# medical-genomics-group/hydra

Hardware: AMD Instinct MI355X
Metric: Gibbs markers/sec/iter (higher is better)
Workload: dtype f64

## Files before the change

### hydra_amd/capi.py

```python
import ctypes as C
import os
import numpy as np

_HERE = os.path.dirname(os.path.abspath(__file__))
LIB_PATH = os.path.join(_HERE, "libhgibbs.so")

ABI_SYMBOLS = [
    "hgibbs_last_error", "hgibbs_version", "hgibbs_create", "hgibbs_destroy", "hgibbs_comm_unique_id",
    "hgibbs_comm_init", "hgibbs_comm_init_external", "hgibbs_p2p_export", "hgibbs_p2p_import", "hgibbs_load_bed", "hgibbs_synth_bed", "hgibbs_dims", "hgibbs_get_bed",
    "hgibbs_marker_stats", "hgibbs_set_residual", "hgibbs_get_residual", "hgibbs_reduce_eps", "hgibbs_add_scalar",
    "hgibbs_update_marker", "hgibbs_dot_marker", "hgibbs_set_covariates", "hgibbs_cov_dot", "hgibbs_cov_update",
    "hydra_chain_set_covariates", "hydra_chain_gamma", "hgibbs_set_components", "hydra_chain_restore",
    "hydra_rng_to_boost_words", "hydra_rng_from_boost_words", "hydra_rng_shuffle", "hgibbs_set_model", "hgibbs_set_beta", "hgibbs_get_beta",
    "hgibbs_beta_sqnorm", "hgibbs_sweep", "hgibbs_set_option", "hgibbs_last_sweep_stats", "hgibbs_stream_ceiling", "hgibbs_debug_times", "hgibbs_resident_trace", "hydra_chain_create",
    "hydra_chain_destroy", "hydra_chain_iterate", "hydra_chain_state", "hydra_chain_csv_line", "hydra_chain_order",
    "hydra_chain_last_nnz", "hgibbs_score", "hgibbs_last_score_ms", "hgibbs_ld", "hgibbs_last_ld_ms",
    "hgibbs_ld_scores", "hgibbs_last_ld_scores_ms",
    "hgibbs_marker_dots", "hgibbs_last_marker_dots_ms", "hgibbs_king", "hgibbs_king_pairs", "hgibbs_king_pairs_get", "hgibbs_last_king_ms",
    "hgibbs_pca", "hgibbs_last_pca_ms", "hgibbs_region_var", "hgibbs_last_region_var_ms",
    "hgibbs_grm", "hgibbs_grm_info", "hgibbs_last_grm_ms",
    "hgibbs_grand_seed", "hgibbs_grand_next", "hgibbs_ars_sample", "hgibbs_w_init", "hgibbs_w_marker_stats", "hgibbs_w_set_model",
    "hgibbs_w_reduce", "hgibbs_w_refresh_vi", "hgibbs_w_get_vi", "hgibbs_w_marker_sums", "hgibbs_w_sweep", "hgibbs_w_last_sweep_stats", "hgibbs_w_ars_device_probe",
    "hgibbs_w_get_beta", "hgibbs_w_set_beta", "hydraw_chain_create", "hydraw_chain_destroy", "hydraw_chain_set_covariates",
    "hydraw_chain_reseed_ars", "hydraw_chain_iterate", "hydraw_chain_state", "hydraw_chain_gamma", "hydraw_chain_order",
    "hydraw_chain_last_nnz", "hydraw_chain_csv_line", "hydraw_chain_restore",
]


class RngState(C.Structure):
    _fields_ = [("x", C.c_uint32 * 624), ("idx", C.c_uint32)]


class SweepStats(C.Structure):
    _fields_ = [("launches", C.c_uint64), ("nnz_updates", C.c_uint64), ("device_ms", C.c_double),
                ("kernel_ms_avg", C.c_double), ("carried_columns", C.c_uint64), ("working_launches", C.c_uint64),
                ("accepted_markers", C.c_uint64), ("streamed_columns", C.c_uint64), ("tiles_per_workgroup_min", C.c_uint32),
                ("tiles_per_workgroup_max", C.c_uint32), ("engine", C.c_uint32), ("walker", C.c_uint32), ("eps_sum_drift", C.c_double),
                ("rounds", C.c_uint64), ("events", C.c_uint64), ("advances", C.c_uint64), ("chunks", C.c_uint64), ("refolds", C.c_uint64), ("pivots", C.c_uint64), ("predicted", C.c_uint64), ("shader_mhz", C.c_double),
                ("ticks", C.c_uint64 * 16), ("refill", C.c_uint32), ("reserved_", C.c_uint32)]


class PcaReport(C.Structure):
    _fields_ = [("iters_run", C.c_int32), ("m_used", C.c_uint32), ("ritz_change", C.c_double), ("resid", C.c_double * 32)]


class RestartState(C.Structure):
    _fields_ = [("iteration", C.c_uint32), ("sigmaE", C.c_double), ("mu", C.c_double),
                ("sigmaG", C.POINTER(C.c_double)), ("estPi", C.POINTER(C.c_double)), ("beta", C.POINTER(C.c_double)),
                ("components", C.POINTER(C.c_int32)), ("eps", C.POINTER(C.c_double)), ("order", C.POINTER(C.c_int32)),
                ("gamma", C.POINTER(C.c_double)), ("xI", C.POINTER(C.c_int32)), ("rng", RngState)]


class GrandState(C.Structure):
    _fields_ = [("r", C.c_int32 * 31), ("f", C.c_int32), ("b", C.c_int32)]


class WSweepStats(C.Structure):
    _fields_ = [("launches", C.c_uint64), ("nnz_updates", C.c_uint64), ("ars_draws", C.c_uint64), ("ars_evals", C.c_uint64),
                ("device_ms", C.c_double), ("sums_kernel_ms", C.c_double)]


class WModelDesc(C.Structure):
# ... 489 lines not shown
        order = np.ascontiguousarray(order, dtype=np.int32)
        sigmaG = np.ascontiguousarray(sigmaG, dtype=np.float64)
        estPi = np.ascontiguousarray(estPi, dtype=np.float64)
        adaV = np.ascontiguousarray(adaV, dtype=np.uint8)
        cass = np.zeros((self.G, self.K), dtype=np.int32)
        nnz = C.c_uint64()
        check(self.L.hgibbs_sweep(self.h, _ip(order), float(sigmaE), _dp(sigmaG), _dp(estPi), _u8(adaV), C.byref(rng),
                                  _ip(cass), C.byref(nnz)))
        return cass, nnz.value

    def resident_trace(self):
        out = np.zeros((10, 4096), dtype=np.uint64)
        check(self.L.hgibbs_resident_trace(self.h, out.ctypes.data_as(C.POINTER(C.c_uint64)), out.size))
        return out

    def sweep_stats(self):
        s = SweepStats()
        check(self.L.hgibbs_last_sweep_stats(self.h, C.byref(s)))
        return {"launches": s.launches, "nnz_updates": s.nnz_updates, "device_ms": s.device_ms,
                "kernel_ms_avg": s.kernel_ms_avg, "carried_columns": s.carried_columns, "working_launches": s.working_launches,
                "accepted_markers": s.accepted_markers, "streamed_columns": s.streamed_columns,
                "tiles_per_workgroup_min": s.tiles_per_workgroup_min, "tiles_per_workgroup_max": s.tiles_per_workgroup_max,
                "engine": s.engine, "walker": s.walker, "refill": s.refill, "eps_sum_drift": s.eps_sum_drift, "rounds": s.rounds, "events": s.events,
                "advances": s.advances, "chunks": s.chunks, "refolds": s.refolds, "pivots": s.pivots, "predicted": s.predicted, "shader_mhz": s.shader_mhz, "ticks": list(s.ticks)}


class Chain:

    def __init__(self, dev, y, mS=None, groups=None, seed=1222, shuffle=1):
        self.dev = dev
        self.L = dev.L
        if mS is None:
            mS = np.array([[0.0, 0.0001, 0.001, 0.01]])
        self.mS = np.ascontiguousarray(mS, dtype=np.float64)
        self.G, self.K = self.mS.shape
        self.groups = None if groups is None else np.ascontiguousarray(groups, dtype=np.int32)
        y = np.ascontiguousarray(y, dtype=np.float64)
        assert y.shape[0] == dev.n_global
        d = ModelDesc(seed, shuffle, self.G, self.K, _ip(self.groups) if self.groups is not None else None, _dp(self.mS))
        self.h = C.c_void_p()
        check(self.L.hydra_chain_create(dev.h, C.byref(d), _dp(y), C.byref(self.h)))
        dev.G, dev.K = self.G, self.K

    def __del__(self):
        try:
            if self.h:
                self.L.hydra_chain_destroy(self.h)
# ... 214 lines not shown
```

### hydra_amd/csrc/hg_resident.hip.h

```cpp
#pragma once

#include "hg_sweep.hip.h"

namespace hg {

constexpr int RS_WAVES = 8;
constexpr int RS_BLOCK = RS_WAVES * WAVE;
constexpr int RS_BMAX = 256;
constexpr int RS_NSH = 8;
constexpr int RS_RSH = 8;
constexpr int RS_GROW = 1024;
constexpr int RS_CROW = 1024;
constexpr int RS_RB = 2 * RS_BMAX;
constexpr int RS_MSG = 16;
constexpr int RS_PMAX = 4;
constexpr int RS_PFIRE = 16;
constexpr int RS_NB = 256;
constexpr int RS_TRACE = 4096;
constexpr int RS_TMAX = 2;
constexpr uint32_t RS_ONE = 1u << 24;
constexpr uint32_t RS_LOW = RS_ONE - 1u;
constexpr unsigned long long RS_ONE64 = 1ull << 56;
constexpr int RS_GFX = 32;
constexpr int RS_FG = 4, RS_FN = 256;
// ... 7 lines not shown
    double dbeta;
};
__host__ __device__ inline uint32_t rs_msg_check(uint32_t seq, uint32_t lo, uint32_t hi)
{
    uint32_t x = seq * 0x9E3779B1u ^ lo ^ (hi * 0x85EBCA77u);
    x ^= x >> 16;
    return x & 0xffffu;
}
constexpr unsigned long long RS_RONE = 1ull << 56;
__host__ __device__ inline unsigned long long rs_raw_value(unsigned long long d) { return (unsigned long long)((long long)(d << 8) >> 8); }
__host__ __device__ inline uint32_t rs_raw_count(unsigned long long d) { return (uint32_t)((d - rs_raw_value(d)) >> 56) & 0xffu; }
__host__ __device__ inline uint32_t rs_window_end(uint32_t C, uint32_t B, uint32_t M, uint32_t mask)
{
    const uint32_t e = (C + B) & ~mask;
    return e < M ? e : M;
}
__host__ __device__ inline uint32_t rs_msg_word0(uint32_t kf, uint32_t ncons, uint32_t seq, uint32_t lo, uint32_t hi) { return (kf << 28) | (rs_msg_check(seq, lo, hi) << 12) | ncons; }

struct ResState {
    uint32_t cursor, rng_idx, error, pad;
    unsigned long long rounds, events, advances, nnz, chunks, refolds, pivots, predicted;
    unsigned long long shader_ticks, wall_ticks;
    unsigned long long t[16];
};

struct ResParams {
    const uint8_t* bed;
    uint64_t stride;
    double* eps;
    uint32_t n_pad, n_local, M;
    double n_minus_1, n_total, eps_sum;
    const int32_t* order;
    const double* s_mave;
    const double* s_mstd;
    const double* s_bold;
    const int32_t* s_ga;
    double* beta;
    int32_t* comp;
    double* acum;
    int32_t* cass;
    int K, GK;
    const double* denom;
    const double* logpi;
    const double* hlog;
    const double* sdk;
    double i_2sigE;
// ... 9 lines not shown
    unsigned long long* racc2;
    unsigned long long* gacc64;
    const unsigned long long* counts;
    unsigned long long* pacc;
    ResMsg* msg;
    ResState* state;
    double fx_scale, fx_unscale;
    unsigned long long timeout;
    unsigned long long* progress;
    unsigned long long rdv_timeout;
    unsigned long long* trace;
    int dbg;
    int pivots;
    int unused_;
    int early_advance;
    uint32_t wend_mask;
    int announce;
    int walker;
    const uint32_t* pred;
    int all_ada;
    int nranks, rank;
    unsigned char* mbox[RX_MAXR];
    unsigned long long sweep_id;
};

constexpr uint32_t RX_RING = 1024;
constexpr size_t RX_GBOX = 0;
constexpr size_t RX_RBOX = RX_GBOX + (size_t)RX_MAXR * 2 * RS_BMAX * 16;
constexpr size_t RX_HBOX = RX_RBOX + (size_t)RX_MAXR * RX_RING * 32;
constexpr size_t RX_BYTES = RX_HBOX + (size_t)RX_MAXR * 2 * 8;
__device__ __forceinline__ unsigned long long* rx_gbox(unsigned char* mb, int src, uint32_t par) { return reinterpret_cast<unsigned long long*>(mb + RX_GBOX) + ((size_t)src * 2 + par) * RS_BMAX * 2; }
__device__ __forceinline__ unsigned long long* rx_rbox(unsigned char* mb, int src) { return reinterpret_cast<unsigned long long*>(mb + RX_RBOX) + (size_t)src * RX_RING * 4; }
__device__ __forceinline__ unsigned long long* rx_hbox(unsigned char* mb, int src) { return reinterpret_cast<unsigned long long*>(mb + RX_HBOX) + (size_t)src * 2; }
__device__ __forceinline__ unsigned long long rx_rtag(unsigned long long sweep, uint32_t batch) { return (0x80000000ull | ((sweep & 0x7ffull) << 20) | (unsigned long long)(batch & 0xfffffu)) << 32; }

typedef uint32_t u4_t __attribute__((ext_vector_type(4)));
typedef __attribute__((address_space(4))) uint32_t rs_cu32;
__device__ __forceinline__ u4_t rs_load16(const void* p)
{
    u4_t v;
    asm volatile("global_load_dwordx4 %0, %1, off sc1\n\ts_waitcnt vmcnt(0)" : "=v"(v) : "v"(p) : "memory");
    return v;
}
__device__ __forceinline__ void rs_lds_barrier() { asm volatile("s_waitcnt lgkmcnt(0)\n\ts_barrier" ::: "memory"); }
__device__ __forceinline__ void rs_store16(void* p, u4_t v) { asm volatile("global_store_dwordx4 %0, %1, off sc1" ::"v"(p), "v"(v) : "memory"); }
__device__ __forceinline__ double rs_readlane(double v, int l)
// ... 403 lines not shown
        last = (kf & RS_LAST) != 0u;
        ncons = (uint32_t)tag & 0xfffu;
        lap(0);
        if (timing) p.trace[4 * RS_TRACE + seq % RS_TRACE] = wall_clock64();
    };
    for (;;) {
        const bool ann = kind == RS_ANNOUNCE;
        const bool upd = kind == RS_EVENT || kind == RS_PIVOT || kind == RS_ANNOUNCED;
        const bool with_gram = kind == RS_EVENT || ann || (kind == RS_ANNOUNCED && !gram_sent);
        if (DBG && wg == 0 && tid == 0) p.progress[1] = ((unsigned long long)seq << 8) | 1u;
        const uint32_t q = C + ncons - 1u;
        const uint32_t Cn = ann ? C : C + ncons;
        const uint32_t Sn = rs_window_end(Cn, B, M, p.wend_mask);
        const uint32_t nnew = Sn - Sx;
        uint32_t count_w = (Sn > (uint32_t)wave ? (Sn - (uint32_t)wave + 7u) / 8u : 0u) - nk;
        cols_landed();

        if (upd || ann) {
            const uint32_t slotq = q & bmask;
            uint32_t xq[T];
#pragma unroll
            for (int t = 0; t < T; ++t) xq[t] = ring[slotq * 64u * T + (uint32_t)lane * T + t];
            const double2 mq = meta[slotq];
            if (upd && tid < 16) {
                const double av = mq.x, sd = mq.y, db = dbeta;
                const double v0 = -(av * sd * db), v1 = db * (1.0 - av) * sd, v2 = db * (2.0 - av) * sd;
                auto addend = [&](uint32_t c) { return 0.0 + ((c == 0u) ? v0 : ((c == 1u) ? v1 : ((c == 3u) ? v2 : 0.0))); };
                tab[tid] = make_double2(addend((uint32_t)tid & 3u), addend(((uint32_t)tid >> 2) & 3u));
            }

            if (with_gram) rs_gram_terms<T, MISS>(p, ring, meta, wg, wave, lane, q, Sx, bmask, nev, xq, mq);
            if (with_gram) ++nev;
            lap(2);
            if (timing) p.trace[6 * RS_TRACE + seq % RS_TRACE] = wall_clock64();
            rs_lds_barrier();
            if (upd) {
#pragma unroll
                for (int t = 0; t < T; ++t) apply_update16_lds(xq[t], tab, e[t]);
                eps_to_lds();
            }
            lap(1);
            if (timing) p.trace[5 * RS_TRACE + seq % RS_TRACE] = wall_clock64();
        }
        gram_sent = ann;
        if (ann) {
            take_message(true);
            if (kind == RS_ABORT) break;
            continue;
        }

        if constexpr (MISS) {
            if (upd) asm volatile("s_waitcnt lgkmcnt(0)\n\ts_barrier" ::: "memory");
        }
        const uint32_t round_k0 = nk;
        uint32_t done_k0 = nk, done_m = 0;
        while (count_w) {
            if (done_m) cols_landed();
            const uint32_t m = count_w < (uint32_t)RS_PF ? count_w : (uint32_t)RS_PF;
            const int32_t ids = rs_lane_ids();
// ... 1315 lines not shown
```

### hydra_amd/csrc/hg_streamer2.hip.h

```cpp
#pragma once

namespace hg {

constexpr int RL_NG = 8;
constexpr int RL_VGPR_LIMIT = 200;
constexpr int RL_VGPR_LIMIT4 = 208;
constexpr int RL_TMAX = 4;
constexpr int RL_EX = 44;
constexpr uint32_t RL_BLK = 144;
typedef int rl_v4i __attribute__((ext_vector_type(4)));

__host__ __device__ constexpr size_t rl_meta_off() { return 512; }
__host__ __device__ constexpr size_t rl_acc_off(uint32_t B) { return 512 + (size_t)B * 16; }
__host__ __device__ constexpr size_t rl_acc2_off(uint32_t B) { return 512 + (size_t)B * 24; }
__host__ __device__ constexpr size_t rl_zero_off(uint32_t B) { return 512 + (size_t)B * 32; }
__host__ __device__ constexpr size_t rl_digit_off(uint32_t B) { return rl_zero_off(B) + 64; }
__host__ __device__ constexpr int rl_image_blocks(int T) { return 8 * T < 16 ? 8 * T : 16; }
__host__ __device__ constexpr size_t rl_ring_off(uint32_t B, int T) { return rl_digit_off(B) + (size_t)RS_WAVES * rl_image_blocks(T) * RL_BLK; }
__host__ __device__ constexpr size_t rl_streamer_lds(uint32_t B, int T) { return rl_ring_off(B, T) + (size_t)B * 256 * T; }
static_assert(rl_streamer_lds(RS_BMAX, RS_TMAX) <= 160 * 1024 && rl_streamer_lds(RS_BMAX / 2, RL_TMAX) <= 160 * 1024,
              "the largest window at the most tiles per workgroup fits the 160 KB of LDS of a compute unit");

#define RL_SET_LIST(X) X(0, 224, 225, 226, 227, 200, 201, 216) X(1, 228, 229, 230, 231, 202, 203, 217) X(2, 232, 233, 234, 235, 204, 205, 218) X(3, 236, 237, 238, 239, 206, 207, 219) \
    X(4, 240, 241, 242, 243, 208, 209, 220) X(5, 244, 245, 246, 247, 210, 211, 221) X(6, 248, 249, 250, 251, 212, 213, 222) X(7, 252, 253, 254, 255, 214, 215, 223)
// ... 312 lines not shown
        ncons = (uint32_t)tag & 0xfffu;
        lap(0);
        if (timing) p.trace[4 * RS_TRACE + seq % RS_TRACE] = wall_clock64();
    };

    for (;;) {
        const bool ann = kind == RS_ANNOUNCE;
        const bool upd = kind == RS_EVENT || kind == RS_PIVOT || kind == RS_ANNOUNCED;
        const bool with_gram = kind == RS_EVENT || ann || (kind == RS_ANNOUNCED && !gram_sent);
        if (DBG && wg == 0 && tid == 0) p.progress[1] = ((unsigned long long)seq << 8) | 1u;
        const uint32_t q = C + ncons - 1u;
        const uint32_t Cn = ann ? C : C + ncons;
        const uint32_t Sn = rs_window_end(Cn, B, M, p.wend_mask);
        const uint32_t nnew = Sn - Sx;
        cols_landed();

        if (upd || ann) {
            const uint32_t slotq = q & bmask;
            uint32_t xq[T];
#pragma unroll
            for (int t = 0; t < T; ++t) xq[t] = ring[slotq * 64u * T + (uint32_t)lane * T + t];
            const uint32_t xqe = ring[slotq * 64u * T + (uint32_t)wave * 8u * T + bw];
            const double2 mq = meta[slotq];
            if (upd && tid < 4) {
                const double av = mq.x, sd = mq.y, db = dbeta;
                const double v0 = -(av * sd * db), v1 = db * (1.0 - av) * sd, v2 = db * (2.0 - av) * sd;
                tab1[tid] = 0.0 + (tid == 0 ? v0 : (tid == 1 ? v1 : (tid == 3 ? v2 : 0.0)));
            }
            if (with_gram) rs_gram_terms<T, MISS>(p, ring, meta, wg, wave, lane, q, Sx, bmask, nev, xq, mq);

            if (with_gram) ++nev;
            lap(2);
            if (timing) p.trace[6 * RS_TRACE + seq % RS_TRACE] = wall_clock64();
            rs_lds_barrier();
            if (upd) {
#pragma unroll
                for (int s = 0; s < ND; ++s) {
                    const double add = tab1[(xqe >> (2u * eb[s])) & 3u];
                    e[s] += ev[s] ? add : 0.0;
                }
                digits_to_operands();
            }
            lap(1);
            if (timing) p.trace[5 * RS_TRACE + seq % RS_TRACE] = wall_clock64();
        }
        gram_sent = ann;
        if (ann) {
            take_message(true);
            if (kind == RS_ABORT) break;
            continue;
        }

        if (nnew) {
            const uint32_t G0 = Sx >> 4, G1 = (Sn - 1u) >> 4;
            for (uint32_t gb = G0; gb <= G1; gb += (uint32_t)NG) {
                if (gb != G0) cols_landed();
                auto one = [&](auto rtag) __attribute__((always_inline)) {
                    constexpr int r = decltype(rtag)::value;
// ... 117 lines not shown
```

### hydra_amd/csrc/hg_walker2.hip.h

```cpp
#pragma once

namespace hg {

constexpr int W2_NBLK = 4;
constexpr uint32_t W2_RING = W2_NBLK * MT_N;
constexpr uint32_t W2_RR = 1024;
constexpr uint32_t W2_EV = 64;
constexpr uint32_t W2_PRED = 1024;
constexpr uint32_t W2_NB = 256;
constexpr int W2_NCH = 4;
constexpr uint32_t W2_NREC = 8;

enum {
    S_FPUB = 0,
    S_MPUB,
    S_CPUB,
    S_SEQPUB,
    S_RECSEQ,
    S_BLK,
    S_GPOS,
    S_PLD,
    S_PCUR,
    S_RDONE,
    S_EVN,
// ... 5 lines not shown
    S_NWORDS = 32
};
enum {
    R_TYPE = 0,
    R_Q,
    R_CN,
    R_SXO,
    R_SXN,
    R_FD,
    R_SEQ,
    R_PIN,
    R_PIQ,
    R_NEV,
    R_GPOSR,
    R_PFN,
    R_DB = 12,
    R_MQ = 14,
    R_SQ = 16,
    R_GSQ = 18,
    R_NMQ = 20,
    R_WORDS = 32
};
enum { RT_EXTEND = 0, RT_ADVANCE = 1, RT_PIVOT = 2, RT_EVENT = 3, RT_END = 4 };
enum { W2_ST_ROUNDS = 0, W2_ST_EVENTS, W2_ST_ADV, W2_ST_NNZ, W2_ST_CHUNKS, W2_ST_REFOLD, W2_ST_PIVOTS, W2_ST_PRED, W2_ST_ANN };

#define W2_ARRAYS(X)                                                                                                                          \
    X(double, tq, (size_t)W2_RING)         \
    X(double, zig_nx, 130)                                                                                                                    \
    X(double, zig_ny, 130)                                                                                                                    \
    X(double, htab, (size_t)4 * HT_LDS)                                                                                                       \
    X(double, qtab, (size_t)2 * HT_LDS)                                                                                                       \
    X(double, ftab, (size_t)RS_FG * (RS_FN + 1))                                                                                              \
    X(double, fscale, RS_FG)                                                                                                                  \
    X(double, mave, MR)                                                                               \
    X(double, mstd, MR)                                                                                                                       \
    X(double, bold, MR)                                                                                                                       \
    X(double, gsum, MR)                                                                                                     \
    X(double, nmis, MR)                                                                                                                       \
    X(double, dpr, Bz)                                                                               \
    X(double, rnum, (size_t)W2_RR)                                                                      \
    X(double, ev_bnew, (size_t)W2_EV)                                                                                                         \
    X(unsigned long long, rprev, (size_t)RS_RB)                                \
    X(unsigned long long, rprev2, (size_t)RS_RB)                                                                                              \
    X(unsigned long long, pprev, (size_t)2 * RS_RB)                                                                                           \
    X(unsigned long long, rloc, Bz)        \
    X(unsigned long long, rloc2, Bz)                                                                       \
    X(uint32_t, rpushed, Bz)                                                                             \
// ... 84 lines not shown
    const Walk2Off off = walk2_offsets(B);
    uint32_t lb = (uint32_t)__builtin_amdgcn_readfirstlane((int)(uint32_t)(uintptr_t)(W2_LDS unsigned char*)hg_smem);
    asm volatile("" : "+s"(lb));
    W2_LDS unsigned char* const lbase = (W2_LDS unsigned char*)(uintptr_t)lb;
#define W2_X(type, name, count) sh.name = (W2_LDS type*)(lbase + off.name);
    W2_ARRAYS(W2_X)
#undef W2_X
    return sh;
}

#define W2_BEXPR pr.B
#define W2_PIVEXPR (pr.pivots != 0)
#define W2_PROLOGUE \
    const int tid = threadIdx.x, lane = tid & 63; \
    const int wave = __builtin_amdgcn_readfirstlane(tid >> 6); \
    const uint32_t B = W2_BEXPR, bmask = B - 1u, M = pr.M; \
    const uint32_t MR = 2u * B, mrmask = MR - 1u; \
    const int K = pr.K, GK = pr.GK; \
    const uint32_t W = pr.W, nsh = pr.nsh, rsh = pr.rsh; \
    const double n_total = pr.n_total, n_minus_1 = pr.n_minus_1, i_2sigE = pr.i_2sigE, eps_sum = pr.eps_sum, fx_unscale = pr.fx_unscale; \
    const unsigned long long timeout = pr.timeout; \
    const bool pivots = W2_PIVEXPR; \
    const uint32_t early_advance = (uint32_t)pr.early_advance; \
    const bool announce = pr.announce != 0 && !pivots; \
    const uint32_t rng_idx0 = pr.rng_idx; \
    ResMsg* const msg = pr.msg; \
    ResState* const state = pr.state; \
    unsigned long long* const trace = pr.trace; \
    unsigned long long* const progress = pr.progress; \
    const uint32_t* const gpred = pr.pred; \
    const double* const zig_ex = pr.zig.ex; \
    const double* const zig_ey = pr.zig.ey; \
    const Walk2Lds sh = walk2_lds(B); \
    const uint32_t cntG[2] = {W / nsh + (W % nsh ? 1u : 0u), W / nsh}; \
    const uint32_t cntR[2] = {W / rsh + (W % rsh ? 1u : 0u), W / rsh}; \
    const uint32_t wend_mask = pr.wend_mask; \
    const int nranks = pr.nranks, rank = pr.rank; \
    const unsigned long long sweep_id = pr.sweep_id; \
    const uint32_t Sx0 = rs_window_end(0u, B, M, wend_mask); \
    const uint32_t m0 = MR < M ? MR : M; \
    auto stage_meta = [&](uint32_t j) { \
        const uint32_t ms = j & mrmask; \
        const int ga = pr.s_ga[j]; \
        const int mk = pr.order[j]; \
        sh.marker[ms] = mk; \
        sh.ga[ms] = ga; \
        sh.bold[ms] = pr.s_bold[j]; \
        sh.mave[ms] = pr.s_mave[j]; \
        sh.mstd[ms] = pr.s_mstd[j]; \
        if constexpr (MISS) { \
            const unsigned long long* cn = pr.counts + 3ull * (unsigned long long)mk; \
            sh.gsum[ms] = (double)(cn[0] + 2ull * cn[1]); \
            sh.nmis[ms] = (double)cn[2]; \
        } \
    }; \
    auto tq_of = [&](uint32_t word) { \
        const double prob = (double)mt_temper(word) * (1.0 / 4294967296.0); \
        return log(1.0 / prob - 1.0) - 1e-9; \
    }; \
    auto aborted = [&]() { return w2_ld(sh.sw + S_ABORT) != 0u; }; \
    auto ended = [&]() { return w2_ld(sh.sw + S_END) != 0u; };

template <int DBG, int MISS, int BC, int RANKS, int DECIDE, int PIV>
__device__ __attribute__((noinline)) void w2_chain(const ResParams& prg)
{
    typedef const __attribute__((address_space(4))) ResParams w2_cparams;
    const unsigned long long pga = (unsigned long long)(uintptr_t)&prg;
    const unsigned long long pgu = ((unsigned long long)(uint32_t)__builtin_amdgcn_readfirstlane((int)(uint32_t)(pga >> 32)) << 32) |
                                   (uint32_t)__builtin_amdgcn_readfirstlane((int)(uint32_t)pga);
    w2_cparams& pr = *(w2_cparams*)(uintptr_t)pgu;
#undef W2_BEXPR
#define W2_BEXPR (BC ? (uint32_t)BC : pr.B)
#undef W2_PIVEXPR
#define W2_PIVEXPR (PIV != 0)
    W2_PROLOGUE
#undef W2_BEXPR
#define W2_BEXPR pr.B
#undef W2_PIVEXPR
#define W2_PIVEXPR (pr.pivots != 0)
    __builtin_amdgcn_s_setprio(3);
    constexpr bool decider = DECIDE != 0;
    const uint32_t nch = B >= 64u ? B / 64u : 1u;
    const uint32_t slot = (uint32_t)wave * 64u + (uint32_t)lane;
    const bool son = slot < B;
    const uint32_t sl = son ? slot : 0u;
    double dpr = 0.0, dp = 0.0, mave = 0.0, mstd = 0.0, boldn = 0.0, fsc = 0.0, gsm = 0.0, nms = 0.0;
    uint32_t fof = 0, sbt = 0, spi = 0;
    bool prd = false;
    uint32_t C = 0, Sx = 0, Fs = 0, base = 0, gposr = rng_idx0 % W2_RING;
    uint32_t gpa32[RS_NSH], gpb32[RS_NSH];
    unsigned long long gpa64[RS_NSH], gpb64[RS_NSH];
#pragma unroll
    for (int r = 0; r < RS_NSH; ++r) {
        gpa32[r] = gpb32[r] = 0u;
        gpa64[r] = gpb64[r] = 0ull;
    }
    typedef const __attribute__((address_space(1))) uint32_t* w2_g32;
    typedef const __attribute__((address_space(1))) unsigned long long* w2_g64;
    const w2_g32 gacc = (w2_g32)pr.gacc;
    const w2_g64 gacc64 = (w2_g64)pr.gacc64;
    uint32_t rno = 0;

    uint32_t seq = 0, nev = 0, pi = 0, evn = 0, pf_n = 0, gpos = rng_idx0, blk = 1u;
    uint32_t rdone_seen = 0, wpub_seen = 0, evw_seen = 0, pld_seen = W2_PRED, fpub_seen = 0, mpub_seen = m0;
    unsigned long long cm[W2_NCH] = {0ull, 0ull, 0ull, 0ull};
    uint32_t stat = 0;
    auto count = [&](uint32_t bits) { stat += (bits >> (uint32_t)lane) & 1u; };
    uint32_t err = 0;
    bool failed = false;
    unsigned long long tacc[8] = {0ull, 0ull, 0ull, 0ull, 0ull, 0ull, 0ull, 0ull};
    unsigned long long tmark = DBG ? wall_clock64() : 0ull;
    auto lap = [&](int i) {
        if (DBG && decider) {
            const unsigned long long now = wall_clock64();
            tacc[i] += now - tmark;
            tmark = now;
        }
    };
    auto pos_of_slot = [&](uint32_t s, uint32_t c) { return c + ((s - c) & bmask); };
    uint32_t nspin = 0;
    auto spin_fail = [&](unsigned long long t0) {
        if (aborted()) return true;
        if (wall_clock64() - t0 > timeout || ((++nspin & 1023u) == 0u && w2_uni((uint32_t)(__hip_atomic_load(progress + 2, HG_RLX_AGENT) != 0ull)) != 0u)) {
            if (lane == 0) w2_st(sh.sw + S_ABORT, 1u);
            return true;
        }
        return false;
// ... 332 lines not shown
                    if ((uint32_t)t <= nch && qs == 0xffffffffu) {
                        uint32_t i = i0 + (uint32_t)t;
                        i = i >= nch ? i - nch : i;
                        unsigned long long mm = i == 0u ? cm[0] : (i == 1u ? cm[1] : (i == 2u ? cm[2] : cm[3]));
                        if (t == 0) mm &= ~lowm;
                        if ((uint32_t)t == nch) mm &= lowm;
                        if (mm) qs = i * 64u + (uint32_t)(__ffsll((long long)mm) - 1);
                    }
                }
                qs = w2_uni(qs);
                if (qs == 0xffffffffu) break;
                const uint32_t qc = pos_of_slot(qs, C);
                const uint32_t qi = qs >> 6, ql = qs & 63u;
                const uint32_t ms = qc & mrmask;
                uint32_t upos = gposr + (qc - C);
                upos = upos >= W2_RING ? upos - W2_RING : upos;
                const double bold_v = sh.bold[ms], num = sh.rnum[qc & (W2_RR - 1u)];
                const double cmq_v = sh.mave[ms], csq_v = sh.mstd[ms], cgsq_v = MISS ? sh.gsum[ms] : 0.0, cnmq_v = MISS ? sh.nmis[ms] : 0.0;
                const int ga_v = sh.ga[ms];
                const uint32_t word_v = sh.mt[upos];
                const uint32_t zp1 = upos + 1u == W2_RING ? 0u : upos + 1u, zp2 = zp1 + 1u == W2_RING ? 0u : zp1 + 1u;
                const uint32_t zw1 = sh.mt[zp1], zw2 = sh.mt[zp2];
                const double bold = w2_uni(bold_v);
                if (announce && !announced && bold != 0.0 && qc + 1u < Sx && (seq + 6u <= (uint32_t)RS_MSG || rdone_seen >= seq + 6u - (uint32_t)RS_MSG)) {
                    if (lane == 0) rs_store16(msg + ((seq + 1u) % RS_MSG), rs_u4(rs_msg_word0((uint32_t)RS_ANNOUNCE, qc - C + 1u, seq + 1u, 0u, 0u), seq + 1u, 0u, 0u));
                    announced = true;
                }
                const uint32_t zleft = blk * (uint32_t)MT_N - (gpos + (qc - C) + 1u);
                double z;
                bool zfast;
                {
                    const uint32_t u1 = mt_temper(w2_uni(zw1)), u2 = mt_temper(w2_uni(zw2));
                    int zi = (int)(u1 & 0xffu);
                    double r = (double)(u1 >> 8) * (1.0 / 16777216.0);
                    r += (double)(u2 & 0x1fffffffu);
                    r *= (1.0 / 536870912.0);
                    const int sign = (zi & 1) * 2 - 1;
                    zi >>= 1;
                    const double x = r * sh.zig_nx[zi];
                    zfast = zleft >= 2u && x < sh.zig_nx[zi + 1];
                    z = x * sign;
                }
                const int g0 = w2_uni(ga_v & 0x0fffffff) * K;
                const double prob = (double)mt_temper(word_v) * (1.0 / 4294967296.0);
                double Lm = 0.0, mk = 0.0, sdl = 0.0;
                {
                    const int lk = lane < K ? lane : 0;
// ... 37 lines not shown
                if (k > 0) {
                    const double mean_k = rs_readlane(mk, k), sd_k = rs_readlane(sdl, k);
                    if (zfast) {
                        bnew = z * sd_k + mean_k;
                        consumed = 2u;
                    } else {
                        if (lane == 0) {
                            RingGen g{sh.mt, zp1, zleft, 0u, 0u};
                            const ZigLds zt{sh.zig_nx, sh.zig_ny, zig_ex, zig_ey};
                            bnew = norm_rng_sd(g, zt, mean_k, sd_k);
                            consumed = g.n;
                            gerr = g.err;
                        }
                        bnew = w2_uni(bnew);
                        consumed = (uint32_t)__builtin_amdgcn_readlane((int)consumed, 0);
                        gerr = (uint32_t)__builtin_amdgcn_readlane((int)gerr, 0);
                    }
                }
                if (gerr) {
                    err = gerr;
                    failed = true;
                    break;
                }
                if (k != 0 || bold != 0.0) {
                    found = true;
                    q_mq = w2_uni(cmq_v);
                    q_sq = w2_uni(csq_v);
                    q_gsq = w2_uni(cgsq_v);
                    q_nmq = w2_uni(cnmq_v);
                    qpos = qc;
                    q_k = k;
                    q_bnew = bnew;
                    q_bold = bold;
                    q_consumed = consumed;
                    break;
                }
                const unsigned long long bit = 1ull << ql;
                if (qi == 0u) cm[0] &= ~bit;
                else if (qi == 1u) cm[1] &= ~bit;
                else if (qi == 2u) cm[2] &= ~bit;
                else cm[3] &= ~bit;
            }
        }
        lap(3);
        if (failed) break;
        const uint32_t early_thr = early_advance;
        const bool early = !found && Fs < Sx && early_thr != 0u && Fs - C >= early_thr;
        if (!found && Fs < Sx && !early) {
            count(1u << W2_ST_REFOLD);
            if (!wait_seen(fpub_seen, S_FPUB, Fs + 1u)) break;
            lap(0);
            publish(RT_EXTEND, 0u, C, Sx, Sx, fpub_seen < Sx ? fpub_seen : Sx, 0u, 0.0, 0.0, 0.0, 0.0, 0.0);
            continue;
        }
        const uint32_t ncons = found ? qpos - C + 1u : (early ? Fs - C : Sx - C);
        const uint32_t Cn = C + ncons;
        const uint32_t Sn = rs_window_end(Cn, B, M, wend_mask);
        const double dbeta = found ? q_bold - q_bnew : 0.0;
        const bool changed = found && dbeta != 0.0;
        const bool is_event = changed || announced;
        const bool predicted = found && q_bold != 0.0;
        bool pivot = false;
        if (PIV && is_event && predicted && pf_n < (uint32_t)RS_PFIRE)
            pivot = qpos + 1u >= Sx || pi - w2_uni(sh.bl_pi[w2_uni(sh.batch[(qpos + 1u) & bmask]) % W2_NB]) < (uint32_t)RS_PMAX;
        lap(6);
        {
            const uint32_t a = w2_uni(fc_rdone), b = w2_uni(fc_wpub), c = w2_uni(fc_evw);
            rdone_seen = a > rdone_seen ? a : rdone_seen;
            wpub_seen = b > wpub_seen ? b : wpub_seen;
            evw_seen = c > evw_seen ? c : evw_seen;
        }
        if (seq + 6u > (uint32_t)RS_MSG && !wait_seen(rdone_seen, S_RDONE, seq + 6u - (uint32_t)RS_MSG)) break;
        if (Cn + B > W2_RR && !wait_seen(wpub_seen, S_WPUB, Cn + B - W2_RR)) break;
        if (evn + 2u > W2_EV && !wait_seen(evw_seen, S_EVW, evn + 2u - W2_EV)) break;
        lap(2);
        ++seq;
        if (lane == 0) {
            const uint32_t kf = (pivot ? (uint32_t)RS_PIVOT : (announced ? (uint32_t)RS_ANNOUNCED : (is_event ? (uint32_t)RS_EVENT : (uint32_t)RS_ADVANCE))) | (Cn >= M ? (uint32_t)RS_LAST : 0u);
            const unsigned long long db = (unsigned long long)__double_as_longlong(dbeta);
            if (DBG) {
                w2_gst(trace + (2 * RS_TRACE + (seq - 1u) % RS_TRACE), wall_clock64());
                w2_gst(trace + (3 * RS_TRACE + (seq - 1u) % RS_TRACE), ncons);
                w2_gst(trace + (0 * RS_TRACE + seq % RS_TRACE), wall_clock64());
                if (!(is_event && !pivot)) w2_gst(trace + (1 * RS_TRACE + seq % RS_TRACE), wall_clock64());
            }
            rs_store16(msg + (seq % RS_MSG), rs_u4(rs_msg_word0(kf, ncons, seq, (uint32_t)db, (uint32_t)(db >> 32)), seq, (uint32_t)db, (uint32_t)(db >> 32)));
        }
        count((1u << W2_ST_ROUNDS) | (is_event ? (1u << W2_ST_EVENTS) | (changed ? 1u << W2_ST_NNZ : 0u) | (predicted ? 1u << W2_ST_PRED : 0u) |
                                                      (announced ? 1u << W2_ST_ANN : 0u)
                                                : 1u << W2_ST_ADV) |
              (pivot ? 1u << W2_ST_PIVOTS : 0u));
        const bool round_trip = is_event && !pivot;
        if (round_trip) ++nev;
        const double mq = q_mq, sq = q_sq, gsq = q_gsq, nmq = q_nmq;
        const uint32_t evr = evn;
        if (found) ++evn;
        const uint32_t piq = pi;
        fpub_seen = w2_ld(sh.sw + S_FPUB);
        const uint32_t Fd = fpub_seen < Sx ? fpub_seen : Sx;
        if (PIV && pivot && Fs < Sx) {
            if (lane == 0) {
                sh.pf_pos[pf_n] = qpos;
                sh.pf_msg[pf_n] = seq;
                sh.pf_pi[pf_n] = pi;
                sh.pf_val[3 * pf_n] = dbeta;
                sh.pf_val[3 * pf_n + 1] = mq;
                sh.pf_val[3 * pf_n + 2] = sq;
            }
            ++pf_n;
        }
        if (PIV && predicted) ++pi;
        gpos += ncons + q_consumed;
        const uint32_t rtype = found ? (pivot ? (uint32_t)RT_PIVOT : (is_event ? (uint32_t)RT_EVENT : (uint32_t)RT_ADVANCE)) : (uint32_t)RT_ADVANCE;
        if (lane == 0) {
// ... 29 lines not shown
        if (C < M) {
            ++seq;
            if (lane == 0) {
                w2_st(sh.sw + S_ABORT, 1u);
                rs_store16(msg + (seq % RS_MSG), rs_u4(rs_msg_word0((uint32_t)RS_ABORT, 0u, seq, 0u, 0u), seq, 0u, 0u));
                atomicMax(&state->error, err ? err : 3u);
            }
        }
        publish(RT_END, 0u, C, Sx, Sx, 0u, 0u, 0.0, 0.0, 0.0, 0.0, 0.0);
        if (lane == 0) {
            w2_st(sh.sw + S_GPOS, gpos);
            w2_lds_done();
            w2_st(sh.sw + S_END, 1u);
            state->cursor = C;
            auto st = [&](int i) { return (uint32_t)__builtin_amdgcn_readlane((int)stat, i); };
            state->rounds = st(W2_ST_ROUNDS);
            state->events = st(W2_ST_EVENTS);
            state->advances = st(W2_ST_ADV);
            state->nnz = st(W2_ST_NNZ);
            state->chunks = st(W2_ST_CHUNKS);
            state->refolds = st(W2_ST_REFOLD);
            state->pivots = st(W2_ST_PIVOTS) + st(W2_ST_ANN);
            state->predicted = st(W2_ST_PRED);
            if (DBG)
                for (int i = 0; i < 8; ++i) state->t[i] = tacc[i];
        }
    }
}

template <int MISS, int RANKS>
__device__ __attribute__((noinline)) void w2_folder(const ResParams& pr)
{
    W2_PROLOGUE
    uint32_t Ff = 0, done = 0, fb = 0;
    unsigned long long t_idle = wall_clock64();
    auto poll_done = [&]() {
        uint32_t b = 0xffffffffu;
        if ((uint32_t)lane < rsh) b = __hip_atomic_load(pr.rcnt + (size_t)lane * RS_CROW, HG_RLX_AGENT) / cntR[(uint32_t)lane < W % rsh ? 0 : 1];
#pragma unroll
        for (int off = 32; off >= 1; off >>= 1) {
            const uint32_t o = (uint32_t)__shfl_xor((int)b, off, 64);
            b = o < b ? o : b;
        }
        done = (uint32_t)__builtin_amdgcn_readfirstlane((int)b);
        if (lane == 0) w2_st(sh.sw + S_RDONE, done);
    };
// ... 378 lines not shown
```

### hydra_amd/csrc/hgibbs.hip

```cpp
#include <hip/hip_runtime.h>
#include <rccl/rccl.h>

#include <algorithm>
#include <atomic>
#include <chrono>
#include <thread>
#include <cmath>
#include <cstdarg>
#include <cstdio>
#include <cstdlib>
#include <cstring>
#include <string>
#include <vector>

#include "../../include/hgibbs.h"
#include "hg_kernels.h"
#include "hg_sweep.hip.h"
#include "hg_resident.hip.h"

using namespace hg;

static thread_local std::string g_err;

static int fail(const char* fmt, ...)
// ... 107 lines not shown
    uint32_t cols_per_group = 4;
    int chunk = 0;
    uint32_t slices = 0;
    uint32_t ext_limit = 256;
    uint32_t max_seg = 0;
    bool gram = true;
    bool use_graph = false;
    bool force_split = false;

    int engine = 0;
    bool res_all_ada = false;
    unsigned long long res_sweep_id = 0;
    bool engine_pinned = false;
    uint32_t window = 0;
    uint32_t res_cus = 0;
    int res_walker = 0;
    bool res_attr_set[20] = {};
    bool res_dead = false;
    uint32_t res_probed_w = 0;
    unsigned long long res_probe_id = 0;
    bool res_not_resident = false;
    int res_early = 24;
    int res_announce = 1;
    int res_wend = 1;
    int res_walker2_ranks = 1;
    double eps_abs_bound = 0.0;
    int res_refill = 0;
    int res_pivots = 0;
    unsigned char* res_acc = nullptr;
    ResMsg* res_msg = nullptr;
    ResState* res_state = nullptr;
    ResState* res_state_host = nullptr;
    ResParams* res_params = nullptr;
    ResParams* res_params_host = nullptr;
    unsigned long long* res_progress = nullptr;
    unsigned long long* res_progress_host = nullptr;
    hipStream_t aux_stream = nullptr;
    unsigned long long* res_trace = nullptr;
    double res_timeout_s = 2.0;
    double res_deadline_s = 0.0;

    hgibbs_sweep_stats stats{};
    int score_sp = 0;
    int score_ranges = 0;
    double score_ms = 0.0;
    int ld_split = 0;
// ... 1082 lines not shown
    } else if (!std::strcmp(name, "ahead")) {
        if (value < -1 || value > AHEAD_MAX) return fail("ahead must be in [-1,%d] (-1 = auto)", AHEAD_MAX);
        h->ahead = (int)value;

    } else if (!std::strcmp(name, "engine")) {
        if (value < 0 || value > 2) return fail("engine must be 0 (auto), 1 (batch) or 2 (resident)");
        h->engine = (int)value;
    } else if (!std::strcmp(name, "window")) {
        if (value != 0 && (value < 8 || value > RS_BMAX || (value & (value - 1)))) return fail("window must be 0 (auto) or a power of two in [8,%d]", RS_BMAX);
        h->window = (uint32_t)value;
    } else if (!std::strcmp(name, "pivots")) {
        h->res_pivots = value != 0;
    } else if (!std::strcmp(name, "early_advance")) {
        if (value < 0 || value > 255) return fail("early_advance must be in [0,255]");
        h->res_early = (int)value;
    } else if (!std::strcmp(name, "refill")) {
        if (value < 0 || value > 2) return fail("refill must be 0 (auto), 1 (fused multiply-adds) or 2 (integer matrix products)");
        h->res_refill = (int)value;
    } else if (!std::strcmp(name, "walker2_ranks")) {
        h->res_walker2_ranks = value != 0;
    } else if (!std::strcmp(name, "window_end16")) {
        h->res_wend = value != 0;
    } else if (!std::strcmp(name, "announce")) {
        h->res_announce = value != 0;
    } else if (!std::strcmp(name, "walker")) {
        if (value < 0 || value > 2) return fail("walker must be 0 (auto), 1 (first) or 2 (second)");
        h->res_walker = (int)value;
    } else if (!std::strcmp(name, "res_cus")) {
        if (value < 0 || value > 4096) return fail("res_cus must be in [0,4096]");
        h->res_cus = (uint32_t)value;
    } else if (!std::strcmp(name, "res_deadline_ms")) {
        h->res_deadline_s = (double)value * 1e-3;
    } else if (!std::strcmp(name, "res_timeout_ms")) {
        if (value < 1) return fail("res_timeout_ms must be positive");
        h->res_timeout_s = (double)value * 1e-3;
    } else if (!std::strcmp(name, "p2p")) {
        h->p2p_enabled = value != 0;
    } else if (!std::strcmp(name, "force_split")) {
        h->force_split = value != 0;
    } else if (!std::strcmp(name, "w_kernel_timing")) {
        h->w_kernel_timing = value != 0;
    } else if (!std::strcmp(name, "debug_timing")) {
        h->debug_timing = value != 0;
    } else if (!std::strcmp(name, "chunk")) {
        h->chunk = (int)value;
    } else {
        return fail("hgibbs_set_option: unknown option '%s'", name);
// ... 208 lines not shown
    p.racc2 = reinterpret_cast<unsigned long long*>(h->res_acc + RES_RACC2_OFF);
    p.gacc64 = reinterpret_cast<unsigned long long*>(h->res_acc + RES_RACC2_OFF + RES_RACC_BYTES);
    p.counts = h->counts;
    p.msg = h->res_msg;
    p.state = h->res_state;
    {
        const double bound = 16.0 * std::sqrt(1024.0 * (h->nranks > 1 ? RS_TMAX : pl.T) * std::max(r0[1], 1e-300)) + 1.0;
        int ex = 50 - (int)std::ceil(std::log2(bound));
        ex = std::max(-40, std::min(ex, 60));
        p.fx_scale = std::ldexp(1.0, ex);
        p.fx_unscale = std::ldexp(1.0, -ex);
    }
    p.timeout = (unsigned long long)(h->res_timeout_s * 1e8);
    p.rdv_timeout = (unsigned long long)(std::min(h->res_timeout_s, 0.1) * 1e8);
    p.dbg = h->debug_timing ? 1 : 0;
    p.pivots = pl.pivots;
    p.nranks = h->nranks > 1 ? h->nranks : 1;
    p.rank = h->nranks > 1 ? h->rank : 0;
    for (int r = 0; r < RX_MAXR; ++r) p.mbox[r] = (h->nranks > 1 && r < h->nranks) ? (unsigned char*)h->peer_base[r] + MBOX_RES_OFF : nullptr;
    p.all_ada = h->res_all_ada ? 1 : 0;
    p.walker = pl.walker;
    p.pred = h->pred;
    p.early_advance = p.nranks > 1 ? 0 : h->res_early;
    p.announce = h->res_announce;
    p.wend_mask = pl.wend_mask;
    {
        const uint32_t nchunk = (h->M + PRED_CHUNK - 1) / PRED_CHUNK;
        k_pred_count<<<nchunk, 256, 0, h->stream>>>(h->s_bold, h->M, h->pred_cnt);
        k_pred_scan<<<1, 1024, 0, h->stream>>>(h->pred_cnt, nchunk);
        k_pred_scatter<<<nchunk, 256, 0, h->stream>>>(h->s_bold, h->M, h->pred_cnt, nchunk, h->pred, nullptr);
        HIP_TRY(hipGetLastError());
    }
    p.sweep_id = ++h->res_sweep_id;
    p.trace = h->res_trace;
    p.progress = h->res_progress;
    HIP_TRY(hipMemsetAsync(h->res_progress, 0, 16 * sizeof(unsigned long long), h->stream));

    HIP_TRY(hipMemsetAsync(h->res_acc, 0, RES_ACC_BYTES, h->stream));
    HIP_TRY(hipMemsetAsync(h->res_msg, 0, RS_MSG * sizeof(ResMsg), h->stream));
    HIP_TRY(hipMemsetAsync(h->res_state, 0, sizeof(ResState), h->stream));
    if (res_opt_in(h, pl)) return 1;
    {
        if (h->occ_kern != (const void*)pl.kern || h->occ_lds != pl.lds) {
            HIP_TRY(hipOccupancyMaxActiveBlocksPerMultiprocessor(&h->occ_per_cu, pl.kern, RS_BLOCK, pl.lds));
            h->occ_kern = (const void*)pl.kern;
            h->occ_lds = pl.lds;
        }
// ... 74 lines not shown
    std::memcpy(rng->x, h->sweep_io_host, MT_N * sizeof(uint32_t));
    if (cass_host) std::memcpy(cass_host, h->sweep_io_host + MT_N, (size_t)h->G * h->K * sizeof(int32_t));
    if (nnz_updates) *nnz_updates = st.nnz;
    hgibbs_sweep_stats& s = h->stats;
    s = hgibbs_sweep_stats{};
    s.launches = 1;
    s.nnz_updates = st.nnz;
    s.device_ms = ms;
    s.working_launches = st.rounds;
    s.kernel_ms_avg = st.rounds ? ms / (double)st.rounds : 0.0;
    s.accepted_markers = st.cursor;
    s.streamed_columns = h->M;
    s.tiles_per_workgroup_min = s.tiles_per_workgroup_max = (uint32_t)pl.T;
    s.engine = 2;
    s.walker = (uint32_t)pl.walker;
    s.refill = (uint32_t)pl.refill;
    s.rounds = st.rounds;
    s.events = st.events;
    s.advances = st.advances;
    s.chunks = st.chunks;
    s.refolds = st.refolds;
    s.pivots = st.pivots;
    s.predicted = st.predicted;
    for (int i = 0; i < 16; ++i) s.ticks[i] = st.t[i];
    s.shader_mhz = st.wall_ticks ? 100.0 * (double)st.shader_ticks / (double)st.wall_ticks : 0.0;
    {
        double r1[2];
        if (reduce_eps_all(h, r1)) return 1;
        s.eps_sum_drift = std::fabs(r1[0] - r0[0]);
    }
    if (timing) {
        auto ms = [](auto a, auto b) { return std::chrono::duration<double, std::milli>(b - a).count(); };
        std::fprintf(stderr, "[hgibbs] resident sweep: launch preparation %.3f ms, kernel wait %.3f ms (device %.3f), results + drift %.3f\n", ms(t_0, t_launch), ms(t_launch, t_kernel),
                     (double)s.device_ms, ms(t_kernel, std::chrono::steady_clock::now()));
    }
    return 0;
}

struct BatchBuild {
    uint32_t cpg;
    int tier, mg, nomiss, dbg;
    void (*kern)(SweepParams);
    void (*draw)(SweepParams);
};
static const BatchBuild BATCH_BUILDS[] = {
    {2, 2, 0, 0, 0, k_sweep_batch<2, 2, 0>, k_sweep_draw<2, 0>},
// ... 306 lines not shown
```

### include/hgibbs.h

```cpp
#ifndef HGIBBS_H
#define HGIBBS_H

#include <stddef.h>
#include <stdint.h>

#ifdef __cplusplus
extern "C" {
#endif

typedef struct hgibbs_ctx* hgibbs_t;

typedef struct {
    uint32_t x[624];
    uint32_t idx;
} hgibbs_rng_state;

const char* hgibbs_last_error(void);
int hgibbs_version(void);

int hgibbs_create(int device_id, hgibbs_t* out);
int hgibbs_destroy(hgibbs_t h);

int hgibbs_comm_unique_id(void* id128);
int hgibbs_comm_init(hgibbs_t h, int nranks, int rank, const void* id128);
// ... 37 lines not shown

int hgibbs_set_option(hgibbs_t h, const char* name, int64_t value);
typedef struct {
    uint64_t launches;
    uint64_t nnz_updates;
    double device_ms;
    double kernel_ms_avg;
    uint64_t carried_columns;
    uint64_t working_launches;
    uint64_t accepted_markers;
    uint64_t streamed_columns;
    uint32_t tiles_per_workgroup_min;
    uint32_t tiles_per_workgroup_max;
    uint32_t engine;
    uint32_t walker;
    double eps_sum_drift;
    uint64_t rounds, events, advances, chunks, refolds;
    uint64_t pivots;
    uint64_t predicted;
    double shader_mhz;
    uint64_t ticks[16];
    uint32_t refill;
    uint32_t reserved_;
} hgibbs_sweep_stats;
int hgibbs_last_sweep_stats(hgibbs_t h, hgibbs_sweep_stats* out);
int hgibbs_stream_ceiling(hgibbs_t h, uint64_t bytes, int reps, double* gbps);
int hgibbs_debug_times(hgibbs_t h, uint64_t* out48);
int hgibbs_resident_trace(hgibbs_t h, uint64_t* out, uint64_t words);

int hgibbs_score(hgibbs_t h, int S, const double* a, const double* o, double* out);
int hgibbs_last_score_ms(hgibbs_t h, double* ms);

int hgibbs_region_var(hgibbs_t h, int S, const double* a, const double* o, uint32_t nsets, const uint64_t* off, const uint32_t* idx,
                      double* mean, double* var);
int hgibbs_last_region_var_ms(hgibbs_t h, double* ms);

int hgibbs_ld(hgibbs_t h, uint32_t m0, uint32_t count, uint32_t W, double* r_host, int64_t* sums_host);
int hgibbs_last_ld_ms(hgibbs_t h, double* ms);

int hgibbs_ld_scores(hgibbs_t h, uint32_t W, const uint32_t* ahead, uint32_t C, const uint64_t* annot, int adjust, double* l2);
int hgibbs_last_ld_scores_ms(hgibbs_t h, double* products_ms, double* reduce_ms);

int hgibbs_marker_dots(hgibbs_t h, uint32_t m0, uint32_t count, int K, const double* U, double* out, double* raw);
int hgibbs_last_marker_dots_ms(hgibbs_t h, double* ms);

int hgibbs_king(hgibbs_t h, uint32_t a0, uint32_t acount, uint32_t b0, uint32_t bcount, int32_t* counts);
// ... 131 lines not shown
```

Measured before the change: 9.139 million.

## Add speculative marker announce mode with auto shut-off and skip zero-delta residual updates

```diff
diff --git a/hydra_amd/capi.py b/hydra_amd/capi.py
--- a/hydra_amd/capi.py
+++ b/hydra_amd/capi.py
@@ -37,7 +37,8 @@
                 ("accepted_markers", C.c_uint64), ("streamed_columns", C.c_uint64), ("tiles_per_workgroup_min", C.c_uint32),
                 ("tiles_per_workgroup_max", C.c_uint32), ("engine", C.c_uint32), ("walker", C.c_uint32), ("eps_sum_drift", C.c_double),
                 ("rounds", C.c_uint64), ("events", C.c_uint64), ("advances", C.c_uint64), ("chunks", C.c_uint64), ("refolds", C.c_uint64), ("pivots", C.c_uint64), ("predicted", C.c_uint64), ("shader_mhz", C.c_double),
-                ("ticks", C.c_uint64 * 16), ("refill", C.c_uint32), ("reserved_", C.c_uint32)]
+                ("ticks", C.c_uint64 * 16), ("refill", C.c_uint32), ("reserved_", C.c_uint32),
+                ("speculated", C.c_uint64), ("speculation_failed", C.c_uint64)]
 
 
 class PcaReport(C.Structure):
@@ -573,7 +574,8 @@
                 "accepted_markers": s.accepted_markers, "streamed_columns": s.streamed_columns,
                 "tiles_per_workgroup_min": s.tiles_per_workgroup_min, "tiles_per_workgroup_max": s.tiles_per_workgroup_max,
                 "engine": s.engine, "walker": s.walker, "refill": s.refill, "eps_sum_drift": s.eps_sum_drift, "rounds": s.rounds, "events": s.events,
-                "advances": s.advances, "chunks": s.chunks, "refolds": s.refolds, "pivots": s.pivots, "predicted": s.predicted, "shader_mhz": s.shader_mhz, "ticks": list(s.ticks)}
+                "advances": s.advances, "chunks": s.chunks, "refolds": s.refolds, "pivots": s.pivots, "predicted": s.predicted, "shader_mhz": s.shader_mhz, "ticks": list(s.ticks),
+                "speculated": s.speculated, "speculation_failed": s.speculation_failed}
 
 
 class Chain:
diff --git a/hydra_amd/csrc/hg_resident.hip.h b/hydra_amd/csrc/hg_resident.hip.h
--- a/hydra_amd/csrc/hg_resident.hip.h
+++ b/hydra_amd/csrc/hg_resident.hip.h
@@ -53,6 +53,7 @@
     unsigned long long rounds, events, advances, nnz, chunks, refolds, pivots, predicted;
     unsigned long long shader_ticks, wall_ticks;
     unsigned long long t[16];
+    unsigned long long speculated, speculation_failed;
 };
 
 struct ResParams {
@@ -108,6 +109,7 @@
     int nranks, rank;
     unsigned char* mbox[RX_MAXR];
     unsigned long long sweep_id;
+    int bound_slack;
 };
 
 constexpr uint32_t RX_RING = 1024;
@@ -557,7 +559,7 @@
 #pragma unroll
             for (int t = 0; t < T; ++t) xq[t] = ring[slotq * 64u * T + (uint32_t)lane * T + t];
             const double2 mq = meta[slotq];
-            if (upd && tid < 16) {
+            if (upd && dbeta != 0.0 && tid < 16) {
                 const double av = mq.x, sd = mq.y, db = dbeta;
                 const double v0 = -(av * sd * db), v1 = db * (1.0 - av) * sd, v2 = db * (2.0 - av) * sd;
                 auto addend = [&](uint32_t c) { return 0.0 + ((c == 0u) ? v0 : ((c == 1u) ? v1 : ((c == 3u) ? v2 : 0.0))); };
@@ -569,7 +571,7 @@
             lap(2);
             if (timing) p.trace[6 * RS_TRACE + seq % RS_TRACE] = wall_clock64();
             rs_lds_barrier();
-            if (upd) {
+            if (upd && dbeta != 0.0) {
 #pragma unroll
                 for (int t = 0; t < T; ++t) apply_update16_lds(xq[t], tab, e[t]);
                 eps_to_lds();
diff --git a/hydra_amd/csrc/hg_streamer2.hip.h b/hydra_amd/csrc/hg_streamer2.hip.h
--- a/hydra_amd/csrc/hg_streamer2.hip.h
+++ b/hydra_amd/csrc/hg_streamer2.hip.h
@@ -358,7 +358,7 @@
             for (int t = 0; t < T; ++t) xq[t] = ring[slotq * 64u * T + (uint32_t)lane * T + t];
             const uint32_t xqe = ring[slotq * 64u * T + (uint32_t)wave * 8u * T + bw];
             const double2 mq = meta[slotq];
-            if (upd && tid < 4) {
+            if (upd && dbeta != 0.0 && tid < 4) {
                 const double av = mq.x, sd = mq.y, db = dbeta;
                 const double v0 = -(av * sd * db), v1 = db * (1.0 - av) * sd, v2 = db * (2.0 - av) * sd;
                 tab1[tid] = 0.0 + (tid == 0 ? v0 : (tid == 1 ? v1 : (tid == 3 ? v2 : 0.0)));
@@ -369,7 +369,7 @@
             lap(2);
             if (timing) p.trace[6 * RS_TRACE + seq % RS_TRACE] = wall_clock64();
             rs_lds_barrier();
-            if (upd) {
+            if (upd && dbeta != 0.0) {
 #pragma unroll
                 for (int s = 0; s < ND; ++s) {
                     const double add = tab1[(xqe >> (2u * eb[s])) & 3u];
diff --git a/hydra_amd/csrc/hg_walker2.hip.h b/hydra_amd/csrc/hg_walker2.hip.h
--- a/hydra_amd/csrc/hg_walker2.hip.h
+++ b/hydra_amd/csrc/hg_walker2.hip.h
@@ -51,7 +51,7 @@
     R_WORDS = 32
 };
 enum { RT_EXTEND = 0, RT_ADVANCE = 1, RT_PIVOT = 2, RT_EVENT = 3, RT_END = 4 };
-enum { W2_ST_ROUNDS = 0, W2_ST_EVENTS, W2_ST_ADV, W2_ST_NNZ, W2_ST_CHUNKS, W2_ST_REFOLD, W2_ST_PIVOTS, W2_ST_PRED, W2_ST_ANN };
+enum { W2_ST_ROUNDS = 0, W2_ST_EVENTS, W2_ST_ADV, W2_ST_NNZ, W2_ST_CHUNKS, W2_ST_REFOLD, W2_ST_PIVOTS, W2_ST_PRED, W2_ST_ANN, W2_ST_SPEC, W2_ST_SPECF };
 
 #define W2_ARRAYS(X)                                                                                                                          \
     X(double, tq, (size_t)W2_RING)         \
@@ -182,7 +182,8 @@
     const unsigned long long timeout = pr.timeout; \
     const bool pivots = W2_PIVEXPR; \
     const uint32_t early_advance = (uint32_t)pr.early_advance; \
-    const bool announce = pr.announce != 0 && !pivots; \
+    const uint32_t announce = pivots ? 0u : (uint32_t)pr.announce; \
+    const double tq_slack = (double)pr.bound_slack; \
     const uint32_t rng_idx0 = pr.rng_idx; \
     ResMsg* const msg = pr.msg; \
     ResState* const state = pr.state; \
@@ -216,7 +217,7 @@
     }; \
     auto tq_of = [&](uint32_t word) { \
         const double prob = (double)mt_temper(word) * (1.0 / 4294967296.0); \
-        return log(1.0 / prob - 1.0) - 1e-9; \
+        return log(1.0 / prob - 1.0) - 1e-9 - tq_slack; \
     }; \
     auto aborted = [&]() { return w2_ld(sh.sw + S_ABORT) != 0u; }; \
     auto ended = [&]() { return w2_ld(sh.sw + S_END) != 0u; };
@@ -263,6 +264,7 @@
 
     uint32_t seq = 0, nev = 0, pi = 0, evn = 0, pf_n = 0, gpos = rng_idx0, blk = 1u;
     uint32_t rdone_seen = 0, wpub_seen = 0, evw_seen = 0, pld_seen = W2_PRED, fpub_seen = 0, mpub_seen = m0;
+    uint32_t ann = announce;
     unsigned long long cm[W2_NCH] = {0ull, 0ull, 0ull, 0ull};
     uint32_t stat = 0;
     auto count = [&](uint32_t bits) { stat += (bits >> (uint32_t)lane) & 1u; };
@@ -641,7 +643,7 @@
                 const uint32_t zp1 = upos + 1u == W2_RING ? 0u : upos + 1u, zp2 = zp1 + 1u == W2_RING ? 0u : zp1 + 1u;
                 const uint32_t zw1 = sh.mt[zp1], zw2 = sh.mt[zp2];
                 const double bold = w2_uni(bold_v);
-                if (announce && !announced && bold != 0.0 && qc + 1u < Sx && (seq + 6u <= (uint32_t)RS_MSG || rdone_seen >= seq + 6u - (uint32_t)RS_MSG)) {
+                if (ann && !announced && (bold != 0.0 || ann >= 2u) && qc + 1u < Sx && (seq + 6u <= (uint32_t)RS_MSG || rdone_seen >= seq + 6u - (uint32_t)RS_MSG)) {
                     if (lane == 0) rs_store16(msg + ((seq + 1u) % RS_MSG), rs_u4(rs_msg_word0((uint32_t)RS_ANNOUNCE, qc - C + 1u, seq + 1u, 0u, 0u), seq + 1u, 0u, 0u));
                     announced = true;
                 }
@@ -725,7 +727,7 @@
                     failed = true;
                     break;
                 }
-                if (k != 0 || bold != 0.0) {
+                if (k != 0 || bold != 0.0 || announced) {
                     found = true;
                     q_mq = w2_uni(cmq_v);
                     q_sq = w2_uni(csq_v);
@@ -763,6 +765,8 @@
         const bool changed = found && dbeta != 0.0;
         const bool is_event = changed || announced;
         const bool predicted = found && q_bold != 0.0;
+        const bool spec = announced && q_bold == 0.0;
+        const bool spec_failed = spec && q_k == 0;
         bool pivot = false;
         if (PIV && is_event && predicted && pf_n < (uint32_t)RS_PFIRE)
             pivot = qpos + 1u >= Sx || pi - w2_uni(sh.bl_pi[w2_uni(sh.batch[(qpos + 1u) & bmask]) % W2_NB]) < (uint32_t)RS_PMAX;
@@ -789,10 +793,15 @@
             }
             rs_store16(msg + (seq % RS_MSG), rs_u4(rs_msg_word0(kf, ncons, seq, (uint32_t)db, (uint32_t)(db >> 32)), seq, (uint32_t)db, (uint32_t)(db >> 32)));
         }
-        count((1u << W2_ST_ROUNDS) | (is_event ? (1u << W2_ST_EVENTS) | (changed ? 1u << W2_ST_NNZ : 0u) | (predicted ? 1u << W2_ST_PRED : 0u) |
-                                                      (announced ? 1u << W2_ST_ANN : 0u)
-                                                : 1u << W2_ST_ADV) |
-              (pivot ? 1u << W2_ST_PIVOTS : 0u));
+        count((1u << W2_ST_ROUNDS) | (spec_failed ? 1u << W2_ST_SPECF
+                                                  : (is_event ? (1u << W2_ST_EVENTS) | (changed ? 1u << W2_ST_NNZ : 0u) | (predicted ? 1u << W2_ST_PRED : 0u) |
+                                                                    (announced ? 1u << W2_ST_ANN : 0u)
+                                                              : 1u << W2_ST_ADV)) |
+              (spec ? 1u << W2_ST_SPEC : 0u) | (pivot ? 1u << W2_ST_PIVOTS : 0u));
+        if (spec_failed && ann == 2u) {
+            const uint32_t nf = (uint32_t)__builtin_amdgcn_readlane((int)stat, W2_ST_SPECF), ns = (uint32_t)__builtin_amdgcn_readlane((int)stat, W2_ST_SPEC);
+            if (nf >= 16u && 4u * nf > ns) ann = 1u;
+        }
         const bool round_trip = is_event && !pivot;
         if (round_trip) ++nev;
         const double mq = q_mq, sq = q_sq, gsq = q_gsq, nmq = q_nmq;
@@ -868,6 +877,8 @@
             state->refolds = st(W2_ST_REFOLD);
             state->pivots = st(W2_ST_PIVOTS) + st(W2_ST_ANN);
             state->predicted = st(W2_ST_PRED);
+            state->speculated = st(W2_ST_SPEC);
+            state->speculation_failed = st(W2_ST_SPECF);
             if (DBG)
                 for (int i = 0; i < 8; ++i) state->t[i] = tacc[i];
         }
diff --git a/hydra_amd/csrc/hgibbs.hip b/hydra_amd/csrc/hgibbs.hip
--- a/hydra_amd/csrc/hgibbs.hip
+++ b/hydra_amd/csrc/hgibbs.hip
@@ -153,6 +153,7 @@
     bool res_not_resident = false;
     int res_early = 24;
     int res_announce = 1;
+    int res_bound_slack = 0;
     int res_wend = 1;
     int res_walker2_ranks = 1;
     double eps_abs_bound = 0.0;
@@ -1281,7 +1282,11 @@
     } else if (!std::strcmp(name, "window_end16")) {
         h->res_wend = value != 0;
     } else if (!std::strcmp(name, "announce")) {
-        h->res_announce = value != 0;
+        if (value < 0 || value > 3) return fail("announce must be 0 (off), 1 (certain events), 2 (first candidates too, with the shut-off) or 3 (without it)");
+        h->res_announce = (int)value;
+    } else if (!std::strcmp(name, "bound_slack")) {
+        if (value < 0 || value > 64) return fail("bound_slack must be in [0,64]");
+        h->res_bound_slack = (int)value;
     } else if (!std::strcmp(name, "walker")) {
         if (value < 0 || value > 2) return fail("walker must be 0 (auto), 1 (first) or 2 (second)");
         h->res_walker = (int)value;
@@ -1536,7 +1541,8 @@
     p.walker = pl.walker;
     p.pred = h->pred;
     p.early_advance = p.nranks > 1 ? 0 : h->res_early;
-    p.announce = h->res_announce;
+    p.announce = p.nranks > 1 ? std::min(h->res_announce, 1) : h->res_announce;
+    p.bound_slack = h->res_bound_slack;
     p.wend_mask = pl.wend_mask;
     {
         const uint32_t nchunk = (h->M + PRED_CHUNK - 1) / PRED_CHUNK;
@@ -1657,6 +1663,8 @@
     s.refolds = st.refolds;
     s.pivots = st.pivots;
     s.predicted = st.predicted;
+    s.speculated = st.speculated;
+    s.speculation_failed = st.speculation_failed;
     for (int i = 0; i < 16; ++i) s.ticks[i] = st.t[i];
     s.shader_mhz = st.wall_ticks ? 100.0 * (double)st.shader_ticks / (double)st.wall_ticks : 0.0;
     {
diff --git a/include/hgibbs.h b/include/hgibbs.h
--- a/include/hgibbs.h
+++ b/include/hgibbs.h
@@ -83,6 +83,8 @@
     uint64_t ticks[16];
     uint32_t refill;
     uint32_t reserved_;
+    uint64_t speculated;
+    uint64_t speculation_failed;
 } hgibbs_sweep_stats;
 int hgibbs_last_sweep_stats(hgibbs_t h, hgibbs_sweep_stats* out);
 int hgibbs_stream_ceiling(hgibbs_t h, uint64_t bytes, int reps, double* gbps);
```

Result: no change. 9.104 million (-0.4%).
